# openclimatefix/predict_pv_yield

Measured on AMD Instinct MI355X. Metric: PV-site samples/sec (train step), conv3d 12->6 frames, higher is better.
Workload: dtype bf16; 1 GPU; conv3d train step (fwd + NMAE + bwd + Adam): sat [B,11,18,64,64] N(0,1), 4x Conv3d(3x3x3, 32ch) + fc 128/128/64, 128.6 M params; per_gpu_batch=32, global_batch=32, t_frames=18, parallelism=single

## Files before the change

include/pv_yield_hip.h:

```cpp
#ifndef PV_YIELD_HIP_H
#define PV_YIELD_HIP_H

#include <stddef.h>
#include <stdint.h>

#ifdef __cplusplus
extern "C" {
#endif

#define PV_ABI_VERSION 1

enum {
  PV_OK = 0,
  PV_EINVAL = -1,
  PV_ESIZE = -2,
  PV_ELAUNCH = -3
};

enum { PV_BORDER_CONSTANT = 0, PV_BORDER_REPLICATE = 1 };

enum {
  PV_U8_ROUND_DIV4 = 0,
  PV_U8_TRUNC_SCALE = 1
};
// ... 228 lines not shown

int pv_linear_f32_skinny_covers(int32_t m, int32_t n, int64_t k);
size_t pv_linear_fwd_f32_skinny_workspace_bytes(int32_t n);
int pv_linear_fwd_f32_skinny(const float* x, const float* w, const float* bias, float* y, int32_t m, int32_t n, int64_t k, int32_t relu,
                             void* workspace, size_t workspace_bytes, void* stream);
int pv_linear_dx_f32_skinny(const float* g, const float* w, float* dx, int32_t m, int32_t n, int64_t k, void* stream);

int pv_linear_workspace_bytes(int32_t m, int32_t n, int64_t k, size_t* bytes);
int pv_linear_fwd_f32(const float* x, const float* w, const float* bias, float* y,
                      int32_t m, int32_t n, int64_t k, int relu,
                      void* workspace, size_t workspace_bytes, void* stream);
int pv_linear_bwd_f32(const float* x, const float* w, const float* dy, const float* y_relu_mask,
                      float* dx, float* dw, float* db,
                      int32_t m, int32_t n, int64_t k, void* stream);

int pv_linear_bf16_workspace_bytes(int32_t m, int32_t n, int64_t k, size_t* bytes);
int pv_linear_fwd_bf16(const uint16_t* x, const uint16_t* w, const float* bias, float* y,
                       int32_t m, int32_t n, int64_t k, int relu,
                       void* workspace, size_t workspace_bytes, void* stream);
int pv_linear_bwd_bf16(const uint16_t* x, const uint16_t* w, const float* dy,
                       const float* y_relu_mask, uint16_t* dx, float* dw, float* db,
                       int32_t m, int32_t n, int64_t k, int32_t gate_dx_by_x, void* stream);

int pv_linear_wgrad_adam_bf16(const uint16_t* x, const float* dy, const float* y_relu_mask, float* param,
                              float* exp_avg, float* exp_avg_sq, uint16_t* bf16_shadow, int32_t m, int32_t n,
                              int64_t k, double lr, double beta1, double beta2, double eps, int32_t step,
                              void* stream);
int pv_linear_wgrad_adam_f32(const float* x, const float* dy, const float* y_relu_mask, float* param, float* exp_avg,
                             float* exp_avg_sq, int32_t m, int32_t n, int64_t k, double lr, double beta1, double beta2,
                             double eps, int32_t step, void* stream);
// ... 158 lines not shown
```

predict_pv_yield_amd/_lib.py:

```python
import ctypes
import os
import subprocess

_PKG = os.path.dirname(os.path.abspath(__file__))
LIB_PATH = os.environ.get("PV_YIELD_LIB") or os.path.join(_PKG, "lib", "libpvyield_hip.so")
CSRC_DIR = os.path.join(_PKG, "csrc")

PV_BORDER_CONSTANT = 0
PV_BORDER_REPLICATE = 1
PV_U8_ROUND_DIV4 = 0
PV_U8_TRUNC_SCALE = 1
PV_OPTFLOW_FARNEBACK_GAUSSIAN = 256

c_i32, c_i64, c_f32, c_f64 = ctypes.c_int32, ctypes.c_int64, ctypes.c_float, ctypes.c_double
c_vp, c_sz, c_int, c_u8 = ctypes.c_void_p, ctypes.c_size_t, ctypes.c_int, ctypes.c_uint8


class FarnebackParams(ctypes.Structure):
    _fields_ = [("pyr_scale", c_f64), ("levels", c_i32), ("winsize", c_i32), ("iterations", c_i32),
                ("poly_n", c_i32), ("poly_sigma", c_f64), ("flags", c_i32)]


class Conv3dDims(ctypes.Structure):
    _fields_ = [("batch", c_i32), ("c_in", c_i32), ("c_out", c_i32), ("t_in", c_i32), ("h_in", c_i32),
                ("w_in", c_i32), ("pad_t", c_i32), ("pad_h", c_i32), ("pad_w", c_i32)]

    def out_shape(self):
        return (self.t_in + 2 * self.pad_t - 2, self.h_in + 2 * self.pad_h - 2, self.w_in + 2 * self.pad_w - 2)


class AdamTensor(ctypes.Structure):
    _fields_ = [("param", c_vp), ("grad", c_vp), ("exp_avg", c_vp), ("exp_avg_sq", c_vp), ("bf16_shadow", c_vp),
                ("n", ctypes.c_uint64)]


class PackJob(ctypes.Structure):
    _fields_ = [("w", c_vp), ("wp", c_vp), ("c_out", c_i32), ("c_in", c_i32), ("transpose_flip", c_i32)]


class GemmDesc(ctypes.Structure):
    _fields_ = [("m", c_i32), ("n", c_i32), ("k", c_i32), ("a_rs", c_i64), ("a_cs", c_i64), ("b_rs", c_i64), ("b_cs", c_i64),
                ("ldc", c_i64), ("batch1", c_i32), ("batch2", c_i32), ("a_bs1", c_i64), ("a_bs2", c_i64), ("b_bs1", c_i64),
                ("b_bs2", c_i64), ("c_bs1", c_i64), ("c_bs2", c_i64), ("k_splits", c_i32), ("c_ss", c_i64)]


class AttentionDesc(ctypes.Structure):
    _fields_ = [("batch", c_i32), ("heads", c_i32), ("n_q", c_i32), ("n_k", c_i32), ("head_dim", c_i32),
                ("q_batch_stride", c_i64), ("q_row_stride", c_i64), ("k_batch_stride", c_i64), ("k_row_stride", c_i64),
                ("scale", c_f32)]


PV_ADAM_MAX_TENSORS = 32
PV_PACK_MAX_JOBS = 16


class Conv3dGeom(ctypes.Structure):
    _fields_ = [(n, c_i32) for n in ("batch", "c_in", "c_out", "t_in", "h_in", "w_in", "k_t", "k_h", "k_w",
                                     "stride_t", "stride_h", "stride_w", "pad_t", "pad_h", "pad_w")]

    def out_shape(self):
        return ((self.t_in + 2 * self.pad_t - self.k_t) // self.stride_t + 1,
                (self.h_in + 2 * self.pad_h - self.k_h) // self.stride_h + 1,
                (self.w_in + 2 * self.pad_w - self.k_w) // self.stride_w + 1)


_PFB = ctypes.POINTER(FarnebackParams)
_PCD = ctypes.POINTER(Conv3dDims)
_PCG = ctypes.POINTER(Conv3dGeom)
# ... 36 lines not shown
    "pv_conv3d_bwd_weight_bf16_workspace_bytes": [_PCD, ctypes.POINTER(c_sz)],
    "pv_conv3d_bwd_weight_bf16": [c_vp, c_vp, c_vp, c_vp, c_vp, _PCD, c_vp, c_sz, c_vp],
    "pv_conv3d_bwd_weight_f16": [c_vp, c_vp, c_vp, c_vp, _PCD, c_vp, c_sz, c_vp],
    "pv_conv3d_split2_weight_elems": [],
    "pv_conv3d_pack_weight_split2_f16": [c_vp, c_vp, c_vp, c_i32, c_i32, c_vp],
    "pv_conv3d_fwd_f16_f32out": [c_vp, c_vp, c_vp, c_i32, _PCD, c_vp],
    "pv_conv3d_fwd_f16_f32out_covers": [_PCD],
    "pv_sum3_ndhwc_to_ncdhw_f32": [c_vp, c_vp, c_vp, c_vp, c_i32, c_vp, c_vp, c_vp, c_vp, c_vp, c_vp, c_i32, c_i32, c_i64, c_vp],
    "pv_linear_f32_skinny_covers": [c_i32, c_i32, c_i64],
    "pv_linear_fwd_f32_skinny_workspace_bytes": [c_i32],
    "pv_linear_fwd_f32_skinny": [c_vp, c_vp, c_vp, c_vp, c_i32, c_i32, c_i64, c_i32, c_vp, c_sz, c_vp],
    "pv_linear_dx_f32_skinny": [c_vp, c_vp, c_vp, c_i32, c_i32, c_i64, c_vp],
    "pv_linear_workspace_bytes": [c_i32, c_i32, c_i64, ctypes.POINTER(c_sz)],
    "pv_linear_fwd_f32": [c_vp, c_vp, c_vp, c_vp, c_i32, c_i32, c_i64, c_int, c_vp, c_sz, c_vp],
    "pv_linear_bwd_f32": [c_vp, c_vp, c_vp, c_vp, c_vp, c_vp, c_vp, c_i32, c_i32, c_i64, c_vp],
    "pv_linear_bf16_workspace_bytes": [c_i32, c_i32, c_i64, ctypes.POINTER(c_sz)],
    "pv_linear_fwd_bf16": [c_vp, c_vp, c_vp, c_vp, c_i32, c_i32, c_i64, c_int, c_vp, c_sz, c_vp],
    "pv_linear_bwd_bf16": [c_vp, c_vp, c_vp, c_vp, c_vp, c_vp, c_vp, c_i32, c_i32, c_i64, c_i32, c_vp],
    "pv_linear_wgrad_adam_bf16": [c_vp, c_vp, c_vp, c_vp, c_vp, c_vp, c_vp, c_i32, c_i32, c_i64, c_f64, c_f64, c_f64, c_f64,
                                  c_i32, c_vp],
    "pv_linear_wgrad_adam_f32": [c_vp, c_vp, c_vp, c_vp, c_vp, c_vp, c_i32, c_i32, c_i64, c_f64, c_f64, c_f64, c_f64, c_i32, c_vp],
    "pv_linear_wgrad_dx_adam_bf16": [c_vp, c_vp, c_vp, c_vp, c_vp, c_vp, c_vp, c_vp, c_vp, c_i32, c_i32, c_i64, c_f64, c_f64,
                                     c_f64, c_f64, c_i32, c_i32, c_i32, c_vp],
    "pv_linear_wgrad_bf16out": [c_vp, c_vp, c_vp, c_vp, c_i32, c_i32, c_i64, c_vp],
    "pv_adam_step_bf16grad": [c_vp, c_vp, c_vp, c_vp, c_vp, c_sz, c_f64, c_f64, c_f64, c_f64, c_i32, c_f32, c_vp],
    "pv_conv3d_general_out_extent": [_PCG, _PI32, _PI32, _PI32],
    "pv_conv3d_general_fwd_f32": [c_vp, c_vp, c_vp, c_vp, _PCG, c_int, c_vp],
    "pv_conv3d_general_bwd_data_f32": [c_vp, c_vp, c_vp, c_vp, c_vp, _PCG, c_vp],
    "pv_conv3d_general_bwd_weight_workspace_bytes": [_PCG, ctypes.POINTER(c_sz)],
    "pv_conv3d_general_bwd_weight_f32": [c_vp, c_vp, c_vp, c_vp, c_vp, _PCG, c_vp, c_sz, c_vp],
# ... 161 lines not shown
```

predict_pv_yield_amd/csrc/dense_f32.hip:

```cpp
#include "pv_common.h"

namespace pv {

__global__ __launch_bounds__(256) void swap01_segments_kernel(const u32x4* __restrict__ src, u32x4* __restrict__ dst, long long n0,
                                                               long long n1, long long seg16) {
  const size_t total = (size_t)n0 * n1 * seg16, stride = (size_t)gridDim.x * blockDim.x;
  for (size_t i = (size_t)blockIdx.x * blockDim.x + threadIdx.x; i < total; i += stride) {
    const size_t seg = i / seg16, c = i - seg * seg16;
    const size_t i1 = seg / n0, i0 = seg - i1 * n0;
    dst[i] = src[(i0 * n1 + i1) * seg16 + c];
  }
}

constexpr int M_TILE = 8;
constexpr long long SMALL_K = 4096, SMALL_MN = 1 << 16;

__global__ __launch_bounds__(256) void linear_fwd_partial_f32(const float* __restrict__ x,
                                                               const float* __restrict__ w,
                                                               float* __restrict__ partial, int m, int n,
                                                               long long k, long long k_chunk) {
  const int col = blockIdx.x;
  const int ks = blockIdx.y;
  const int m0 = blockIdx.z * M_TILE;
  const long long k0 = (long long)ks * k_chunk;
  const long long k1 = k0 + k_chunk < k ? k0 + k_chunk : k;
  float acc[M_TILE];
#pragma unroll
  for (int i = 0; i < M_TILE; ++i) acc[i] = 0.f;
  const float* wr = w + (size_t)col * k;
// ... 105 lines not shown
  for (int ks = 0; ks < k_splits; ++ks) s += partial[(size_t)ks * m * n + i];
  if (bias) s += bias[col];
  if (relu) s = s > 0.f ? s : 0.f;
  y[i] = s;
}

__device__ __forceinline__ void linear_bwd_dx_body(float* g , const float* __restrict__ w,
                                                   const float* __restrict__ dy, const float* __restrict__ ymask,
                                                   float* __restrict__ dx, int m, int n, long long k, int bx, int by) {
  const int m0 = by * M_TILE;
  for (int i = threadIdx.x; i < n * M_TILE; i += blockDim.x) {
    int col = i / M_TILE, r = i % M_TILE;
    float v = 0.f;
    if (m0 + r < m) {
      size_t off = (size_t)(m0 + r) * n + col;
      v = dy[off];
      if (ymask && !(ymask[off] > 0.f)) v = 0.f;
    }
    g[i] = v;
  }
  __syncthreads();
  long long kk = (long long)bx * blockDim.x + threadIdx.x;
  if (kk >= k) return;
  float acc[M_TILE];
#pragma unroll
  for (int i = 0; i < M_TILE; ++i) acc[i] = 0.f;
  int col = 0;
  for (; col + 32 <= n; col += 32) {
    float wv[32];
#pragma unroll
    for (int j = 0; j < 32; ++j) wv[j] = w[(size_t)(col + j) * k + kk];
#pragma unroll
    for (int j = 0; j < 32; ++j)
#pragma unroll
      for (int i = 0; i < M_TILE; ++i) acc[i] = fmaf(g[(col + j) * M_TILE + i], wv[j], acc[i]);
  }
  for (; col + 8 <= n; col += 8) {
    float wv[8];
#pragma unroll
    for (int j = 0; j < 8; ++j) wv[j] = w[(size_t)(col + j) * k + kk];
#pragma unroll
    for (int j = 0; j < 8; ++j)
#pragma unroll
      for (int i = 0; i < M_TILE; ++i) acc[i] = fmaf(g[(col + j) * M_TILE + i], wv[j], acc[i]);
  }
  for (; col < n; ++col) {
    float wv = w[(size_t)col * k + kk];
#pragma unroll
    for (int i = 0; i < M_TILE; ++i) acc[i] = fmaf(g[col * M_TILE + i], wv, acc[i]);
  }
#pragma unroll
  for (int i = 0; i < M_TILE; ++i)
    if (m0 + i < m) dx[(size_t)(m0 + i) * k + kk] = acc[i];
}

__global__ __launch_bounds__(256) void linear_bwd_dx_f32(const float* __restrict__ w, const float* __restrict__ dy,
                                                          const float* __restrict__ ymask, float* __restrict__ dx,
                                                          int m, int n, long long k) {
  extern __shared__ float g[];
  linear_bwd_dx_body(g, w, dy, ymask, dx, m, n, k, blockIdx.x, blockIdx.y);
}

constexpr int N_TILE = 8;
__device__ __forceinline__ void linear_bwd_dw_body(float* g , const float* __restrict__ x,
                                                   const float* __restrict__ dy, const float* __restrict__ ymask,
                                                   float* __restrict__ dw, int m, int n, long long k, int bx, int by) {
  const int n0 = by * N_TILE;
  for (int i = threadIdx.x; i < m * N_TILE; i += blockDim.x) {
    int r = i / N_TILE, j = i % N_TILE;
    float v = 0.f;
    if (n0 + j < n) {
      size_t off = (size_t)r * n + n0 + j;
      v = dy[off];
      if (ymask && !(ymask[off] > 0.f)) v = 0.f;
    }
    g[i] = v;
  }
  __syncthreads();
  long long kk = (long long)bx * blockDim.x + threadIdx.x;
  if (kk >= k) return;
  float acc[N_TILE];
#pragma unroll
  for (int j = 0; j < N_TILE; ++j) acc[j] = 0.f;
  int r = 0;
  for (; r + 32 <= m; r += 32) {
    float xv[32];
#pragma unroll
    for (int q = 0; q < 32; ++q) xv[q] = x[(size_t)(r + q) * k + kk];
#pragma unroll
    for (int q = 0; q < 32; ++q)
#pragma unroll
      for (int j = 0; j < N_TILE; ++j) acc[j] = fmaf(g[(r + q) * N_TILE + j], xv[q], acc[j]);
  }
  for (; r + 8 <= m; r += 8) {
    float xv[8];
#pragma unroll
    for (int q = 0; q < 8; ++q) xv[q] = x[(size_t)(r + q) * k + kk];
#pragma unroll
    for (int q = 0; q < 8; ++q)
#pragma unroll
      for (int j = 0; j < N_TILE; ++j) acc[j] = fmaf(g[(r + q) * N_TILE + j], xv[q], acc[j]);
  }
  for (; r < m; ++r) {
    float xv = x[(size_t)r * k + kk];
#pragma unroll
    for (int j = 0; j < N_TILE; ++j) acc[j] = fmaf(g[r * N_TILE + j], xv, acc[j]);
  }
#pragma unroll
  for (int j = 0; j < N_TILE; ++j)
    if (n0 + j < n) dw[(size_t)(n0 + j) * k + kk] = acc[j];
}

__global__ __launch_bounds__(256) void linear_bwd_dw_f32(const float* __restrict__ x, const float* __restrict__ dy,
                                                          const float* __restrict__ ymask, float* __restrict__ dw,
                                                          int m, int n, long long k) {
  extern __shared__ float g[];
  linear_bwd_dw_body(g, x, dy, ymask, dw, m, n, k, blockIdx.x, blockIdx.y);
}

__device__ __forceinline__ void linear_bwd_db_body(const float* __restrict__ dy, const float* __restrict__ ymask,
                                                   float* __restrict__ db, int m, int n, int bx);

__global__ __launch_bounds__(256) void linear_bwd_db_f32(const float* __restrict__ dy, const float* __restrict__ ymask,
                                                          float* __restrict__ db, int m, int n) {
  linear_bwd_db_body(dy, ymask, db, m, n, blockIdx.x);
}

__device__ __forceinline__ void linear_bwd_db_body(const float* __restrict__ dy, const float* __restrict__ ymask,
                                                   float* __restrict__ db, int m, int n, int bx) {
  int col = bx * blockDim.x + threadIdx.x;
  if (col >= n) return;
  float s = 0.f;
  for (int r = 0; r < m; ++r) {
    size_t off = (size_t)r * n + col;
    float v = dy[off];
    if (ymask && !(ymask[off] > 0.f)) v = 0.f;
    s += v;
  }
  db[col] = s;
}

__global__ __launch_bounds__(256) void linear_bwd_small_f32(const float* __restrict__ x, const float* __restrict__ w,
                                                             const float* __restrict__ dy, const float* __restrict__ ymask,
                                                             float* __restrict__ dx, float* __restrict__ dw,
                                                             float* __restrict__ db, int m, int n, long long k, int kb,
                                                             int n_dx, int n_dw) {
  extern __shared__ float g[];
  int blk = blockIdx.x;
  if (blk < n_dx) {
    linear_bwd_dx_body(g, w, dy, ymask, dx, m, n, k, blk % kb, blk / kb);
  } else if (blk < n_dx + n_dw) {
    blk -= n_dx;
    linear_bwd_dw_body(g, x, dy, ymask, dw, m, n, k, blk % kb, blk / kb);
  } else {
    linear_bwd_db_body(dy, ymask, db, m, n, blk - n_dx - n_dw);
  }
}

__global__ __launch_bounds__(256) void linear_fwd_small_f32(const float* __restrict__ x, const float* __restrict__ w,
                                                             const float* __restrict__ bias, float* __restrict__ y, int m,
                                                             int n, int k, int relu) {
  const int i = blockIdx.x * blockDim.x + threadIdx.x;
  if (i >= m * n) return;
  const int r = i / n, col = i - r * n;
  const float* xr = x + (size_t)r * k;
  const float* wr = w + (size_t)col * k;
  float s0 = 0.f, s1 = 0.f, s2 = 0.f, s3 = 0.f;
  int kk = 0;
  if ((((uintptr_t)xr | (uintptr_t)wr) & 15) == 0) {
    for (; kk + 64 <= k; kk += 64) {
      f32x4 xv[16], wv[16];
#pragma unroll
      for (int j = 0; j < 16; ++j) xv[j] = *reinterpret_cast<const f32x4*>(xr + kk + 4 * j), wv[j] = *reinterpret_cast<const f32x4*>(wr + kk + 4 * j);
#pragma unroll
      for (int j = 0; j < 16; ++j) {
        s0 = fmaf(xv[j][0], wv[j][0], s0);
        s1 = fmaf(xv[j][1], wv[j][1], s1);
        s2 = fmaf(xv[j][2], wv[j][2], s2);
        s3 = fmaf(xv[j][3], wv[j][3], s3);
      }
    }
    for (; kk + 32 <= k; kk += 32) {
      f32x4 xv[8], wv[8];
#pragma unroll
      for (int j = 0; j < 8; ++j) xv[j] = *reinterpret_cast<const f32x4*>(xr + kk + 4 * j), wv[j] = *reinterpret_cast<const f32x4*>(wr + kk + 4 * j);
#pragma unroll
      for (int j = 0; j < 8; ++j) {
        s0 = fmaf(xv[j][0], wv[j][0], s0);
        s1 = fmaf(xv[j][1], wv[j][1], s1);
        s2 = fmaf(xv[j][2], wv[j][2], s2);
        s3 = fmaf(xv[j][3], wv[j][3], s3);
      }
    }
  }
  for (; kk + 4 <= k; kk += 4) {
    s0 = fmaf(xr[kk], wr[kk], s0);
    s1 = fmaf(xr[kk + 1], wr[kk + 1], s1);
    s2 = fmaf(xr[kk + 2], wr[kk + 2], s2);
    s3 = fmaf(xr[kk + 3], wr[kk + 3], s3);
  }
  for (; kk < k; ++kk) s0 = fmaf(xr[kk], wr[kk], s0);
  float s = (s0 + s1) + (s2 + s3);
  if (bias) s += bias[col];
  if (relu) s = s > 0.f ? s : 0.f;
  y[i] = s;
}

struct LossWeights { float w[64]; };

__global__ __launch_bounds__(256) void forecast_losses_f32(const float* __restrict__ y_hat, const float* __restrict__ y,
                                                            long long y_row_stride, long long y_col_stride, int m,
                                                            int n, float grad_scale, LossWeights lw,
                                                            float* __restrict__ out4, float* __restrict__ grad,
                                                            float* __restrict__ per_horizon) {
  float s_se = 0.f, s_ae = 0.f, s_wse = 0.f, s_wae = 0.f;
  const int total = m * n;
  const float inv = 1.0f / (float)total;
  for (int i = threadIdx.x; i < total; i += blockDim.x) {
    int r = i / n, c = i - r * n;
    float d = y_hat[i] - y[(long long)r * y_row_stride + (long long)c * y_col_stride];
// ... 480 lines not shown
```

predict_pv_yield_amd/functional.py:

```python
import ctypes

import torch

from . import hip_ops as K
from ._lib import check, current_stream_ptr, get_lib, ptr


LINEAR_F32_GEMM_K = 1 << 16
F32_PENDING_MAX_ROWS = 1024


def exact_f32() -> bool:
    import os
    return bool(os.environ.get("PV_EXACT_F32"))


class LinearF32(torch.autograd.Function):
    @staticmethod
    def forward(ctx, x, weight, bias, relu):
        x = x.contiguous()
        if (not exact_f32() and x.dtype == torch.float32 and weight.is_contiguous()
                and K.linear_f32_skinny_covers(x.shape[0], weight.shape[0], x.shape[1])):
            y = K.linear_fwd_f32_skinny(x, weight, bias.contiguous() if bias is not None else None, relu)
        else:
# ... 24 lines not shown
                dw = None
            else:
                if earlier is not None:
                    x0, g0 = earlier
                    owner._pv_pending_f32 = None
                    dw0 = K.gemm(g0.t(), x0)
                    owner.grad = dw0 if owner.grad is None else owner.grad + dw0
                dw = K.gemm(g.t(), x)
            return dx, dw, (K.colsum(g) if ctx.has_bias else None), None
        dx, dw, db = K.linear_bwd_f32(x, weight.contiguous(), dy.contiguous(), y, need_dx=ctx.needs_input_grad[0])
        return dx, dw, (db if ctx.has_bias else None), None


def linear_f32(x, weight, bias, relu=False):
    return LinearF32.apply(x, weight, bias, relu)


USE_RELU_MASKS = True


class PackInputBF16(torch.autograd.Function):

    @staticmethod
    def forward(ctx, x):
        out = K.pack_ncdhw_f32_to_ndhwc_bf16(x.contiguous())
        ctx.mark_non_differentiable(out)
        return out

    @staticmethod
    def backward(ctx, g):
# ... 566 lines not shown
```

predict_pv_yield_amd/hip_ops.py:

```python
import ctypes
from typing import Optional, Sequence

import numpy as np
import torch

from . import _lib
from ._lib import (Conv3dDims, Conv3dGeom, FarnebackParams, PV_BORDER_CONSTANT, PV_BORDER_REPLICATE,
                   PV_OPTFLOW_FARNEBACK_GAUSSIAN, check, current_stream_ptr, get_lib, ptr, require_cuda)

c_i32, c_i64, c_f32, c_f64, c_sz = ctypes.c_int32, ctypes.c_int64, ctypes.c_float, ctypes.c_double, ctypes.c_size_t


def u8_from_10bit(x: torch.Tensor, mode: int = 0, return_flag: bool = False):
    require_cuda(x)
    out = torch.empty(x.shape, dtype=torch.uint8, device=x.device)
    flag = torch.zeros(1, dtype=torch.int32, device=x.device)
    lib = get_lib()
    if x.dtype == torch.int16:
        fn = lib.pv_u8_from_10bit_i16
    elif x.dtype == torch.float32:
        fn = lib.pv_u8_from_10bit_f32
    else:
        raise TypeError(f"u8_from_10bit: int16 or float32 expected, got {x.dtype}")
    check(fn(ptr(x), ptr(out), x.numel(), mode, ptr(flag), current_stream_ptr()), "pv_u8_from_10bit")
# ... 557 lines not shown
    dx = torch.empty((m, k), dtype=torch.float32, device=g.device)
    check(get_lib().pv_linear_dx_f32_skinny(ptr(g), ptr(weight), ptr(dx), m, n, k, current_stream_ptr()), "pv_linear_dx_f32_skinny")
    return dx


def linear_bwd_f32(x, weight, dy, y_mask, need_dx=True):
    require_cuda(x, weight, dy, y_mask)
    m, k = x.shape
    n = weight.shape[0]
    dx = torch.empty((m, k), dtype=torch.float32, device=x.device) if need_dx else None
    dw = torch.empty((n, k), dtype=torch.float32, device=x.device)
    db = torch.empty(n, dtype=torch.float32, device=x.device)
    check(get_lib().pv_linear_bwd_f32(ptr(x), ptr(weight), ptr(dy), ptr(y_mask), ptr(dx), ptr(dw), ptr(db), m, n, k,
                                      current_stream_ptr()), "pv_linear_bwd_f32")
    return dx, dw, db


LINEAR_FWD_MAX_ROWS = 1024


def linear_fwd_bf16(x_bf16, w_bf16, bias, relu=False):
    require_cuda(x_bf16, w_bf16, bias)
    m, k = x_bf16.shape
    n = w_bf16.shape[0]
    need = c_sz(0)
    lib = get_lib()
    cap = LINEAR_FWD_MAX_ROWS if (32 <= n <= 128 and n % 16 == 0) else 128
    check(lib.pv_linear_bf16_workspace_bytes(min(m, cap), n, k, ctypes.byref(need)), "pv_linear_bf16_workspace_bytes")
    ws = _workspace("linear_bf16", need.value, x_bf16.device)
    y = torch.empty((m, n), dtype=torch.float32, device=x_bf16.device)
# ... 1214 lines not shown
```

predict_pv_yield_amd/models/conv3d/model.py:

```python
import logging

import torch
from torch import nn

from ...data.batch import BatchML
from ..base_model import BaseModel

logging.basicConfig()
_LOG = logging.getLogger("predict_pv_yield_amd")


FC1_CHANNELS_LAST = True


class Model(BaseModel):

    name = "conv3d"

    def __init__(
        self,
        include_pv_yield: bool = True,
        include_nwp: bool = True,
        forecast_minutes: int = 30,
        history_minutes: int = 60,
# ... 102 lines not shown
            return replace_future_frames_with_flow(sat.float(), n_future=self.forecast_len_5)
        return sat.float()

    def forward(self, x):
        if type(x) == dict:
            x = BatchML(**x)
        sat_data = self._satellite_input(x)
        from ... import functional as Fn
        from ._tower import conv_tower_fc1
        self._mark_fc1_layout()

        batch_size = sat_data.shape[0]
        out = conv_tower_fc1(sat_data, self._conv_layers(), self.fc1, self.number_sat_channels, self.conv3d_channels,
                             (0, 0, 0), self.cnn_output_size, self.precision == "bf16" and self._bf16_supported(),
                             fc1_channels_last=bool(self._fc1_k_channels))
        out = Fn.linear_f32(out, self.fc2.weight, self.fc2.bias, relu=True)

        if self.include_pv_yield:
            pv_yield_history = x[self.output_variable][:, : self.history_len_30 + 1].nan_to_num(nan=0.0).float()
            pv_yield_history = pv_yield_history.reshape(pv_yield_history.shape[0],
                                                        pv_yield_history.shape[1] * pv_yield_history.shape[2])
            out = torch.cat((out, pv_yield_history), dim=1)
        if self.include_nwp:
            nwp_data = x["nwp"].float().flatten(start_dim=1)
            out_nwp = Fn.linear_f32(nwp_data, self.fc_nwp.weight, self.fc_nwp.bias, relu=True)
            out = torch.cat((out, out_nwp), dim=1)

        out = Fn.linear_f32(out, self.fc3.weight, self.fc3.bias, relu=True)
        out = Fn.linear_f32(out, self.fc4.weight, self.fc4.bias, relu=False)
        return out.reshape(batch_size, self.forecast_len)
# ... 1 lines not shown
```

Measured before the change: 20330 samples/s.

## Fuse fc2/fc3/fc4 MLP head into single forward and backward kernels

Adds fused HIP kernels that run the three small fp32 linear layers after fc1 in one launch for the forward pass and one for the backward pass. Activations stay in LDS between layers, and the backward kernel computes the dx chain, dw and db tiles together. The goal is to cut per-layer kernel-launch and autograd overhead for the tiny batch-32 head. The model uses this path only when neither PV-yield history nor NWP inputs are included, and it falls back to per-layer linears when the shapes do not fit in LDS. The existing dense kernels are refactored into shared device bodies.

New measurement: 20620 samples/s (median of 6 runs). 1.01x the previous value.

```diff
diff --git a/include/pv_yield_hip.h b/include/pv_yield_hip.h
--- a/include/pv_yield_hip.h
+++ b/include/pv_yield_hip.h
@@ -266,6 +266,21 @@
                       float* dx, float* dw, float* db,
                       int32_t m, int32_t n, int64_t k, void* stream);
 
+#define PV_MLP_HEAD_MAX_LAYERS 3
+typedef struct pv_mlp_layer {
+  const float* w;
+  const float* bias;
+  float* y;
+  float* dw;
+  float* db;
+  int32_t n;
+  int32_t relu;
+} pv_mlp_layer;
+int pv_mlp_head_max_rows(int32_t k1, const int32_t* n, int32_t n_layers);
+int pv_mlp_head_fwd_f32(const float* x, int32_t m, int32_t k1, const pv_mlp_layer* layers, int32_t n_layers, void* stream);
+int pv_mlp_head_bwd_f32(const float* x, const float* dy, float* dx, int32_t m, int32_t k1, const pv_mlp_layer* layers,
+                        int32_t n_layers, void* stream);
+
 int pv_linear_bf16_workspace_bytes(int32_t m, int32_t n, int64_t k, size_t* bytes);
 int pv_linear_fwd_bf16(const uint16_t* x, const uint16_t* w, const float* bias, float* y,
                        int32_t m, int32_t n, int64_t k, int relu,
diff --git a/predict_pv_yield_amd/_lib.py b/predict_pv_yield_amd/_lib.py
--- a/predict_pv_yield_amd/_lib.py
+++ b/predict_pv_yield_amd/_lib.py
@@ -38,6 +38,10 @@
     _fields_ = [("w", c_vp), ("wp", c_vp), ("c_out", c_i32), ("c_in", c_i32), ("transpose_flip", c_i32)]
 
 
+class MlpLayer(ctypes.Structure):
+    _fields_ = [("w", c_vp), ("bias", c_vp), ("y", c_vp), ("dw", c_vp), ("db", c_vp), ("n", c_i32), ("relu", c_i32)]
+
+
 class GemmDesc(ctypes.Structure):
     _fields_ = [("m", c_i32), ("n", c_i32), ("k", c_i32), ("a_rs", c_i64), ("a_cs", c_i64), ("b_rs", c_i64), ("b_cs", c_i64),
                 ("ldc", c_i64), ("batch1", c_i32), ("batch2", c_i32), ("a_bs1", c_i64), ("a_bs2", c_i64), ("b_bs1", c_i64),
@@ -52,6 +56,7 @@
 
 PV_ADAM_MAX_TENSORS = 32
 PV_PACK_MAX_JOBS = 16
+PV_MLP_HEAD_MAX_LAYERS = 3
 
 
 class Conv3dGeom(ctypes.Structure):
@@ -118,6 +123,9 @@
     "pv_linear_workspace_bytes": [c_i32, c_i32, c_i64, ctypes.POINTER(c_sz)],
     "pv_linear_fwd_f32": [c_vp, c_vp, c_vp, c_vp, c_i32, c_i32, c_i64, c_int, c_vp, c_sz, c_vp],
     "pv_linear_bwd_f32": [c_vp, c_vp, c_vp, c_vp, c_vp, c_vp, c_vp, c_i32, c_i32, c_i64, c_vp],
+    "pv_mlp_head_max_rows": [c_i32, _PI32, c_i32],
+    "pv_mlp_head_fwd_f32": [c_vp, c_i32, c_i32, ctypes.POINTER(MlpLayer), c_i32, c_vp],
+    "pv_mlp_head_bwd_f32": [c_vp, c_vp, c_vp, c_i32, c_i32, ctypes.POINTER(MlpLayer), c_i32, c_vp],
     "pv_linear_bf16_workspace_bytes": [c_i32, c_i32, c_i64, ctypes.POINTER(c_sz)],
     "pv_linear_fwd_bf16": [c_vp, c_vp, c_vp, c_vp, c_i32, c_i32, c_i64, c_int, c_vp, c_sz, c_vp],
     "pv_linear_bwd_bf16": [c_vp, c_vp, c_vp, c_vp, c_vp, c_vp, c_vp, c_i32, c_i32, c_i64, c_i32, c_vp],
diff --git a/predict_pv_yield_amd/csrc/dense_f32.hip b/predict_pv_yield_amd/csrc/dense_f32.hip
--- a/predict_pv_yield_amd/csrc/dense_f32.hip
+++ b/predict_pv_yield_amd/csrc/dense_f32.hip
@@ -1,4 +1,5 @@
 #include "pv_common.h"
+#include "dense_f32_bodies.h"
 
 namespace pv {
 
@@ -12,7 +13,6 @@
   }
 }
 
-constexpr int M_TILE = 8;
 constexpr long long SMALL_K = 4096, SMALL_MN = 1 << 16;
 
 __global__ __launch_bounds__(256) void linear_fwd_partial_f32(const float* __restrict__ x,
@@ -148,8 +148,7 @@
     float v = 0.f;
     if (m0 + r < m) {
       size_t off = (size_t)(m0 + r) * n + col;
-      v = dy[off];
-      if (ymask && !(ymask[off] > 0.f)) v = 0.f;
+      v = linear_bwd_gate(dy[off], ymask, off);
     }
     g[i] = v;
   }
@@ -157,32 +156,7 @@
   long long kk = (long long)bx * blockDim.x + threadIdx.x;
   if (kk >= k) return;
   float acc[M_TILE];
-#pragma unroll
-  for (int i = 0; i < M_TILE; ++i) acc[i] = 0.f;
-  int col = 0;
-  for (; col + 32 <= n; col += 32) {
-    float wv[32];
-#pragma unroll
-    for (int j = 0; j < 32; ++j) wv[j] = w[(size_t)(col + j) * k + kk];
-#pragma unroll
-    for (int j = 0; j < 32; ++j)
-#pragma unroll
-      for (int i = 0; i < M_TILE; ++i) acc[i] = fmaf(g[(col + j) * M_TILE + i], wv[j], acc[i]);
-  }
-  for (; col + 8 <= n; col += 8) {
-    float wv[8];
-#pragma unroll
-    for (int j = 0; j < 8; ++j) wv[j] = w[(size_t)(col + j) * k + kk];
-#pragma unroll
-    for (int j = 0; j < 8; ++j)
-#pragma unroll
-      for (int i = 0; i < M_TILE; ++i) acc[i] = fmaf(g[(col + j) * M_TILE + i], wv[j], acc[i]);
-  }
-  for (; col < n; ++col) {
-    float wv = w[(size_t)col * k + kk];
-#pragma unroll
-    for (int i = 0; i < M_TILE; ++i) acc[i] = fmaf(g[col * M_TILE + i], wv, acc[i]);
-  }
+  linear_bwd_dx_acc<M_TILE>(g, M_TILE, w, n, k, kk, acc);
 #pragma unroll
   for (int i = 0; i < M_TILE; ++i)
     if (m0 + i < m) dx[(size_t)(m0 + i) * k + kk] = acc[i];
@@ -195,7 +169,6 @@
   linear_bwd_dx_body(g, w, dy, ymask, dx, m, n, k, blockIdx.x, blockIdx.y);
 }
 
-constexpr int N_TILE = 8;
 __device__ __forceinline__ void linear_bwd_dw_body(float* g , const float* __restrict__ x,
                                                    const float* __restrict__ dy, const float* __restrict__ ymask,
                                                    float* __restrict__ dw, int m, int n, long long k, int bx, int by) {
@@ -205,8 +178,7 @@
     float v = 0.f;
     if (n0 + j < n) {
       size_t off = (size_t)r * n + n0 + j;
-      v = dy[off];
-      if (ymask && !(ymask[off] > 0.f)) v = 0.f;
+      v = linear_bwd_gate(dy[off], ymask, off);
     }
     g[i] = v;
   }
@@ -214,32 +186,7 @@
   long long kk = (long long)bx * blockDim.x + threadIdx.x;
   if (kk >= k) return;
   float acc[N_TILE];
-#pragma unroll
-  for (int j = 0; j < N_TILE; ++j) acc[j] = 0.f;
-  int r = 0;
-  for (; r + 32 <= m; r += 32) {
-    float xv[32];
-#pragma unroll
-    for (int q = 0; q < 32; ++q) xv[q] = x[(size_t)(r + q) * k + kk];
-#pragma unroll
-    for (int q = 0; q < 32; ++q)
-#pragma unroll
-      for (int j = 0; j < N_TILE; ++j) acc[j] = fmaf(g[(r + q) * N_TILE + j], xv[q], acc[j]);
-  }
-  for (; r + 8 <= m; r += 8) {
-    float xv[8];
-#pragma unroll
-    for (int q = 0; q < 8; ++q) xv[q] = x[(size_t)(r + q) * k + kk];
-#pragma unroll
-    for (int q = 0; q < 8; ++q)
-#pragma unroll
-      for (int j = 0; j < N_TILE; ++j) acc[j] = fmaf(g[(r + q) * N_TILE + j], xv[q], acc[j]);
-  }
-  for (; r < m; ++r) {
-    float xv = x[(size_t)r * k + kk];
-#pragma unroll
-    for (int j = 0; j < N_TILE; ++j) acc[j] = fmaf(g[r * N_TILE + j], xv, acc[j]);
-  }
+  linear_bwd_dw_acc(g, x, m, k, kk, acc);
 #pragma unroll
   for (int j = 0; j < N_TILE; ++j)
     if (n0 + j < n) dw[(size_t)(n0 + j) * k + kk] = acc[j];
@@ -264,14 +211,10 @@
                                                    float* __restrict__ db, int m, int n, int bx) {
   int col = bx * blockDim.x + threadIdx.x;
   if (col >= n) return;
-  float s = 0.f;
-  for (int r = 0; r < m; ++r) {
-    size_t off = (size_t)r * n + col;
-    float v = dy[off];
-    if (ymask && !(ymask[off] > 0.f)) v = 0.f;
-    s += v;
-  }
-  db[col] = s;
+  db[col] = linear_bwd_db_sum(m, [&](int r) {
+    const size_t off = (size_t)r * n + col;
+    return linear_bwd_gate(dy[off], ymask, off);
+  });
 }
 
 __global__ __launch_bounds__(256) void linear_bwd_small_f32(const float* __restrict__ x, const float* __restrict__ w,
@@ -299,45 +242,7 @@
   const int r = i / n, col = i - r * n;
   const float* xr = x + (size_t)r * k;
   const float* wr = w + (size_t)col * k;
-  float s0 = 0.f, s1 = 0.f, s2 = 0.f, s3 = 0.f;
-  int kk = 0;
-  if ((((uintptr_t)xr | (uintptr_t)wr) & 15) == 0) {
-    for (; kk + 64 <= k; kk += 64) {
-      f32x4 xv[16], wv[16];
-#pragma unroll
-      for (int j = 0; j < 16; ++j) xv[j] = *reinterpret_cast<const f32x4*>(xr + kk + 4 * j), wv[j] = *reinterpret_cast<const f32x4*>(wr + kk + 4 * j);
-#pragma unroll
-      for (int j = 0; j < 16; ++j) {
-        s0 = fmaf(xv[j][0], wv[j][0], s0);
-        s1 = fmaf(xv[j][1], wv[j][1], s1);
-        s2 = fmaf(xv[j][2], wv[j][2], s2);
-        s3 = fmaf(xv[j][3], wv[j][3], s3);
-      }
-    }
-    for (; kk + 32 <= k; kk += 32) {
-      f32x4 xv[8], wv[8];
-#pragma unroll
-      for (int j = 0; j < 8; ++j) xv[j] = *reinterpret_cast<const f32x4*>(xr + kk + 4 * j), wv[j] = *reinterpret_cast<const f32x4*>(wr + kk + 4 * j);
-#pragma unroll
-      for (int j = 0; j < 8; ++j) {
-        s0 = fmaf(xv[j][0], wv[j][0], s0);
-        s1 = fmaf(xv[j][1], wv[j][1], s1);
-        s2 = fmaf(xv[j][2], wv[j][2], s2);
-        s3 = fmaf(xv[j][3], wv[j][3], s3);
-      }
-    }
-  }
-  for (; kk + 4 <= k; kk += 4) {
-    s0 = fmaf(xr[kk], wr[kk], s0);
-    s1 = fmaf(xr[kk + 1], wr[kk + 1], s1);
-    s2 = fmaf(xr[kk + 2], wr[kk + 2], s2);
-    s3 = fmaf(xr[kk + 3], wr[kk + 3], s3);
-  }
-  for (; kk < k; ++kk) s0 = fmaf(xr[kk], wr[kk], s0);
-  float s = (s0 + s1) + (s2 + s3);
-  if (bias) s += bias[col];
-  if (relu) s = s > 0.f ? s : 0.f;
-  y[i] = s;
+  y[i] = linear_fwd_epilogue_f32(linear_fwd_dot_f32(xr, wr, k), bias, col, relu);
 }
 
 struct LossWeights { float w[64]; };
diff --git a/predict_pv_yield_amd/csrc/dense_f32_bodies.h b/predict_pv_yield_amd/csrc/dense_f32_bodies.h
--- /dev/null
+++ b/predict_pv_yield_amd/csrc/dense_f32_bodies.h
@@ -0,0 +1,126 @@
+#pragma once
+#include "pv_common.h"
+
+namespace pv {
+
+constexpr int M_TILE = 8;
+constexpr int N_TILE = 8;
+
+__device__ __forceinline__ float linear_fwd_dot_f32(const float* __restrict__ xr, const float* __restrict__ wr, int k) {
+  float s0 = 0.f, s1 = 0.f, s2 = 0.f, s3 = 0.f;
+  int kk = 0;
+  if ((((uintptr_t)xr | (uintptr_t)wr) & 15) == 0) {
+    for (; kk + 64 <= k; kk += 64) {
+      f32x4 xv[16], wv[16];
+#pragma unroll
+      for (int j = 0; j < 16; ++j) xv[j] = *reinterpret_cast<const f32x4*>(xr + kk + 4 * j), wv[j] = *reinterpret_cast<const f32x4*>(wr + kk + 4 * j);
+#pragma unroll
+      for (int j = 0; j < 16; ++j) {
+        s0 = fmaf(xv[j][0], wv[j][0], s0);
+        s1 = fmaf(xv[j][1], wv[j][1], s1);
+        s2 = fmaf(xv[j][2], wv[j][2], s2);
+        s3 = fmaf(xv[j][3], wv[j][3], s3);
+      }
+    }
+    for (; kk + 32 <= k; kk += 32) {
+      f32x4 xv[8], wv[8];
+#pragma unroll
+      for (int j = 0; j < 8; ++j) xv[j] = *reinterpret_cast<const f32x4*>(xr + kk + 4 * j), wv[j] = *reinterpret_cast<const f32x4*>(wr + kk + 4 * j);
+#pragma unroll
+      for (int j = 0; j < 8; ++j) {
+        s0 = fmaf(xv[j][0], wv[j][0], s0);
+        s1 = fmaf(xv[j][1], wv[j][1], s1);
+        s2 = fmaf(xv[j][2], wv[j][2], s2);
+        s3 = fmaf(xv[j][3], wv[j][3], s3);
+      }
+    }
+  }
+  for (; kk + 4 <= k; kk += 4) {
+    s0 = fmaf(xr[kk], wr[kk], s0);
+    s1 = fmaf(xr[kk + 1], wr[kk + 1], s1);
+    s2 = fmaf(xr[kk + 2], wr[kk + 2], s2);
+    s3 = fmaf(xr[kk + 3], wr[kk + 3], s3);
+  }
+  for (; kk < k; ++kk) s0 = fmaf(xr[kk], wr[kk], s0);
+  return (s0 + s1) + (s2 + s3);
+}
+
+__device__ __forceinline__ float linear_fwd_epilogue_f32(float s, const float* __restrict__ bias, int col, int relu) {
+  if (bias) s += bias[col];
+  if (relu) s = s > 0.f ? s : 0.f;
+  return s;
+}
+
+__device__ __forceinline__ float linear_bwd_gate(float dy, const float* __restrict__ ymask, size_t off) {
+  return (ymask && !(ymask[off] > 0.f)) ? 0.f : dy;
+}
+
+template <int R>
+__device__ __forceinline__ void linear_bwd_dx_acc(const float* g, int g_stride, const float* __restrict__ w, int n, long long k,
+                                                  long long kk, float (&acc)[R]) {
+#pragma unroll
+  for (int i = 0; i < R; ++i) acc[i] = 0.f;
+  int col = 0;
+  for (; col + 32 <= n; col += 32) {
+    float wv[32];
+#pragma unroll
+    for (int j = 0; j < 32; ++j) wv[j] = w[(size_t)(col + j) * k + kk];
+#pragma unroll
+    for (int j = 0; j < 32; ++j)
+#pragma unroll
+      for (int i = 0; i < R; ++i) acc[i] = fmaf(g[(col + j) * g_stride + i], wv[j], acc[i]);
+  }
+  for (; col + 8 <= n; col += 8) {
+    float wv[8];
+#pragma unroll
+    for (int j = 0; j < 8; ++j) wv[j] = w[(size_t)(col + j) * k + kk];
+#pragma unroll
+    for (int j = 0; j < 8; ++j)
+#pragma unroll
+      for (int i = 0; i < R; ++i) acc[i] = fmaf(g[(col + j) * g_stride + i], wv[j], acc[i]);
+  }
+  for (; col < n; ++col) {
+    float wv = w[(size_t)col * k + kk];
+#pragma unroll
+    for (int i = 0; i < R; ++i) acc[i] = fmaf(g[col * g_stride + i], wv, acc[i]);
+  }
+}
+
+__device__ __forceinline__ void linear_bwd_dw_acc(const float* g, const float* __restrict__ x, int m, long long k, long long kk,
+                                                  float (&acc)[N_TILE]) {
+#pragma unroll
+  for (int j = 0; j < N_TILE; ++j) acc[j] = 0.f;
+  int r = 0;
+  for (; r + 32 <= m; r += 32) {
+    float xv[32];
+#pragma unroll
+    for (int q = 0; q < 32; ++q) xv[q] = x[(size_t)(r + q) * k + kk];
+#pragma unroll
+    for (int q = 0; q < 32; ++q)
+#pragma unroll
+      for (int j = 0; j < N_TILE; ++j) acc[j] = fmaf(g[(r + q) * N_TILE + j], xv[q], acc[j]);
+  }
+  for (; r + 8 <= m; r += 8) {
+    float xv[8];
+#pragma unroll
+    for (int q = 0; q < 8; ++q) xv[q] = x[(size_t)(r + q) * k + kk];
+#pragma unroll
+    for (int q = 0; q < 8; ++q)
+#pragma unroll
+      for (int j = 0; j < N_TILE; ++j) acc[j] = fmaf(g[(r + q) * N_TILE + j], xv[q], acc[j]);
+  }
+  for (; r < m; ++r) {
+    float xv = x[(size_t)r * k + kk];
+#pragma unroll
+    for (int j = 0; j < N_TILE; ++j) acc[j] = fmaf(g[r * N_TILE + j], xv, acc[j]);
+  }
+}
+
+template <class G>
+__device__ __forceinline__ float linear_bwd_db_sum(int m, G g_at) {
+  float s = 0.f;
+  for (int r = 0; r < m; ++r) s += g_at(r);
+  return s;
+}
+
+}
diff --git a/predict_pv_yield_amd/csrc/mlp_head_f32.hip b/predict_pv_yield_amd/csrc/mlp_head_f32.hip
--- /dev/null
+++ b/predict_pv_yield_amd/csrc/mlp_head_f32.hip
@@ -0,0 +1,239 @@
+#include "pv_common.h"
+#include "dense_f32_bodies.h"
+
+namespace pv {
+
+constexpr int HEAD_MAX_LAYERS = PV_MLP_HEAD_MAX_LAYERS;
+constexpr int HEAD_MAX_WIDTH = 4096;
+constexpr int HEAD_DX_ROWS = 2;
+constexpr long long HEAD_MAX_MN = 1 << 16;
+constexpr size_t HEAD_MAX_LDS = 64 * 1024;
+
+struct HeadArgs {
+  pv_mlp_layer layer[HEAD_MAX_LAYERS];
+  int n_layers;
+};
+
+__global__ __launch_bounds__(256) void mlp_head_fwd_f32_kernel(const float* __restrict__ x, HeadArgs a, int m, int k1,
+                                                               int rows_per_wg, int ws) {
+  extern __shared__ __attribute__((aligned(16))) float head_lds[];
+  const int r0 = blockIdx.x * rows_per_wg;
+  const int rows = m - r0 < rows_per_wg ? m - r0 : rows_per_wg;
+  float* cur = head_lds;
+  float* nxt = head_lds + (size_t)rows_per_wg * ws;
+  for (int i = threadIdx.x; i < rows * k1; i += blockDim.x) {
+    const int r = i / k1, c = i - r * k1;
+    cur[r * ws + c] = x[(size_t)(r0 + r) * k1 + c];
+  }
+  __syncthreads();
+  int k = k1;
+  for (int l = 0; l < a.n_layers; ++l) {
+    const pv_mlp_layer L = a.layer[l];
+    for (int i = threadIdx.x; i < rows * L.n; i += blockDim.x) {
+      const int r = i / L.n, col = i - r * L.n;
+      const float s = linear_fwd_epilogue_f32(linear_fwd_dot_f32(cur + r * ws, L.w + (size_t)col * k, k), L.bias, col, L.relu);
+      L.y[(size_t)(r0 + r) * L.n + col] = s;
+      nxt[r * ws + col] = s;
+    }
+    __syncthreads();
+    float* t = cur; cur = nxt; nxt = t;
+    k = L.n;
+  }
+}
+
+template <class Out>
+__device__ __forceinline__ void head_dx_stage(const float* G, int n, const float* __restrict__ w, int k, int rows, int c0, int cn,
+                                              Out out) {
+  for (int it = threadIdx.x; it < rows * cn; it += blockDim.x) {
+    const int r = it / cn, kk = c0 + (it - r * cn);
+    float acc[1];
+    linear_bwd_dx_acc<1>(G + (size_t)r * n, 1, w, n, (long long)k, (long long)kk, acc);
+    out(r, kk, acc[0]);
+  }
+}
+
+__device__ __forceinline__ const float* head_mask(const pv_mlp_layer& L) { return L.relu ? L.y : nullptr; }
+
+__device__ __forceinline__ const float* head_g_chain(const HeadArgs& a, const float* __restrict__ dy, int ra, int rows, int stop,
+                                                     float* Ga, float* Gb) {
+  const int last = a.n_layers - 1;
+  {
+    const pv_mlp_layer L = a.layer[last];
+    const float* mask = head_mask(L);
+    for (int i = threadIdx.x; i < rows * L.n; i += blockDim.x) {
+      const size_t off = (size_t)ra * L.n + i;
+      Ga[i] = linear_bwd_gate(dy[off], mask, off);
+    }
+  }
+  __syncthreads();
+  for (int j = last; j > stop; --j) {
+    const pv_mlp_layer L = a.layer[j], P = a.layer[j - 1];
+    const float* mask = head_mask(P);
+    float* Gout = Gb;
+    head_dx_stage(Ga, L.n, L.w, P.n, rows, 0, P.n, [&](int r, int kk, float v) {
+      Gout[r * P.n + kk] = linear_bwd_gate(v, mask, (size_t)(ra + r) * P.n + kk);
+    });
+    __syncthreads();
+    float* t = Ga; Ga = Gb; Gb = t;
+  }
+  return Ga;
+}
+
+struct HeadBwdPlan {
+  int n_dx;
+  int tile0[HEAD_MAX_LAYERS + 1];
+  int kb[HEAD_MAX_LAYERS];
+  int g_floats;
+};
+
+__global__ __launch_bounds__(256) void mlp_head_bwd_f32_kernel(const float* __restrict__ x, const float* __restrict__ dy,
+                                                               float* __restrict__ dx, HeadArgs a, HeadBwdPlan p, int m, int k1) {
+  extern __shared__ __attribute__((aligned(16))) float head_lds[];
+  float* Ga = head_lds;
+  float* Gb = head_lds + p.g_floats;
+  float* gt = head_lds + 2 * (size_t)p.g_floats;
+  const int blk = blockIdx.x;
+  if (blk < p.n_dx) {
+    const int ra = blk * HEAD_DX_ROWS;
+    const int rows = m - ra < HEAD_DX_ROWS ? m - ra : HEAD_DX_ROWS;
+    const float* G = head_g_chain(a, dy, ra, rows, 0, Ga, Gb);
+    const pv_mlp_layer L = a.layer[0];
+    head_dx_stage(G, L.n, L.w, k1, rows, 0, k1, [&](int r, int kk, float v) { dx[(size_t)(ra + r) * k1 + kk] = v; });
+    return;
+  }
+  int t = 0;
+  while (t + 1 < a.n_layers && blk - p.n_dx >= p.tile0[t + 1]) ++t;
+  const pv_mlp_layer L = a.layer[t];
+  const int tile = blk - p.n_dx - p.tile0[t];
+  const int bx = tile % p.kb[t], n0 = (tile / p.kb[t]) * N_TILE;
+  const int k = t == 0 ? k1 : a.layer[t - 1].n;
+  const float* xin = t == 0 ? x : a.layer[t - 1].y;
+  const float* mask = head_mask(L);
+  if (t == a.n_layers - 1) {
+    for (int i = threadIdx.x; i < m * N_TILE; i += blockDim.x) {
+      const int r = i / N_TILE, j = i % N_TILE;
+      float v = 0.f;
+      if (n0 + j < L.n) {
+        const size_t off = (size_t)r * L.n + n0 + j;
+        v = linear_bwd_gate(dy[off], mask, off);
+      }
+      gt[i] = v;
+    }
+  } else {
+    const float* G = head_g_chain(a, dy, 0, m, t + 1, Ga, Gb);
+    const pv_mlp_layer U = a.layer[t + 1];
+    const int cn = L.n - n0 < N_TILE ? L.n - n0 : N_TILE;
+    if (cn < N_TILE)
+      for (int i = threadIdx.x; i < m * N_TILE; i += blockDim.x)
+        if (i % N_TILE >= cn) gt[i] = 0.f;
+    head_dx_stage(G, U.n, U.w, L.n, m, n0, cn, [&](int r, int kk, float v) {
+      gt[r * N_TILE + (kk - n0)] = linear_bwd_gate(v, mask, (size_t)r * L.n + kk);
+    });
+  }
+  __syncthreads();
+  if (bx == 0 && threadIdx.x < N_TILE && n0 + (int)threadIdx.x < L.n) {
+    const int j = threadIdx.x;
+    L.db[n0 + j] = linear_bwd_db_sum(m, [&](int r) { return gt[r * N_TILE + j]; });
+  }
+  const long long kk = (long long)bx * blockDim.x + threadIdx.x;
+  if (kk >= k) return;
+  float acc[N_TILE];
+  linear_bwd_dw_acc(gt, xin, m, (long long)k, kk, acc);
+#pragma unroll
+  for (int j = 0; j < N_TILE; ++j)
+    if (n0 + j < L.n) L.dw[(size_t)(n0 + j) * k + kk] = acc[j];
+}
+
+static int head_args(const pv_mlp_layer* layers, int32_t n_layers, int32_t m, int32_t k1, HeadArgs* a, const char* who) {
+  PV_REQUIRE(layers && n_layers >= 1 && n_layers <= HEAD_MAX_LAYERS, PV_EINVAL, "%s: 1..%d layers", who, HEAD_MAX_LAYERS);
+  PV_REQUIRE(m > 0 && k1 > 0 && k1 <= HEAD_MAX_WIDTH, PV_ESIZE, "%s: m > 0 and k1 in 1..%d, got %d x %d", who, HEAD_MAX_WIDTH, m, k1);
+  a->n_layers = n_layers;
+  for (int l = 0; l < n_layers; ++l) {
+    PV_REQUIRE(layers[l].w && layers[l].y, PV_EINVAL, "%s: null weight / output of layer %d", who, l);
+    PV_REQUIRE(layers[l].n > 0 && layers[l].n <= HEAD_MAX_WIDTH, PV_ESIZE, "%s: layer %d has %d outputs (1..%d)", who, l,
+               layers[l].n, HEAD_MAX_WIDTH);
+    PV_REQUIRE((long long)m * layers[l].n <= HEAD_MAX_MN, PV_ESIZE, "%s: %d rows x %d outputs of layer %d is no small layer", who, m,
+               layers[l].n, l);
+    a->layer[l] = layers[l];
+  }
+  return PV_OK;
+}
+
+static size_t head_bwd_g_floats(const HeadArgs& a, int m) {
+  int wide_all = 0, wide_upper = 0;
+  for (int l = 0; l < a.n_layers; ++l) {
+    wide_all = std::max(wide_all, a.layer[l].n);
+    if (l > 0) wide_upper = std::max(wide_upper, a.layer[l].n);
+  }
+  return (std::max((size_t)m * wide_upper, (size_t)HEAD_DX_ROWS * wide_all) + 3) & ~(size_t)3;
+}
+
+}
+
+using namespace pv;
+
+extern "C" {
+
+int pv_mlp_head_max_rows(int32_t k1, const int32_t* n, int32_t n_layers) {
+  if (!n || n_layers < 1 || n_layers > HEAD_MAX_LAYERS || k1 < 1 || k1 > HEAD_MAX_WIDTH) return 0;
+  HeadArgs a;
+  a.n_layers = n_layers;
+  for (int l = 0; l < n_layers; ++l) {
+    if (n[l] < 1 || n[l] > HEAD_MAX_WIDTH) return 0;
+    a.layer[l].n = n[l];
+  }
+  int wide = 1;
+  for (int l = 0; l < n_layers; ++l) wide = std::max(wide, n[l]);
+  int lo = 0, hi = (int)(HEAD_MAX_MN / wide);
+  while (lo < hi) {
+    const int mid = (lo + hi + 1) / 2;
+    if ((2 * head_bwd_g_floats(a, mid) + (size_t)mid * N_TILE) * sizeof(float) <= HEAD_MAX_LDS) lo = mid; else hi = mid - 1;
+  }
+  return lo;
+}
+
+int pv_mlp_head_fwd_f32(const float* x, int32_t m, int32_t k1, const pv_mlp_layer* layers, int32_t n_layers, void* stream) {
+  HeadArgs a;
+  const int rc = head_args(layers, n_layers, m, k1, &a, "pv_mlp_head_fwd_f32");
+  if (rc) return rc;
+  PV_REQUIRE(x, PV_EINVAL, "pv_mlp_head_fwd_f32: null x");
+  int wide = k1;
+  for (int l = 0; l < n_layers; ++l) wide = std::max(wide, a.layer[l].n);
+  const int ws = (wide + 3) & ~3;
+  const int rows_per_wg = (m + kNumCU - 1) / kNumCU;
+  const size_t lds = 2 * (size_t)rows_per_wg * ws * sizeof(float);
+  PV_REQUIRE(lds <= HEAD_MAX_LDS, PV_ESIZE, "pv_mlp_head_fwd_f32: %d rows of %d features do not fit the LDS image", m, wide);
+  const unsigned threads = (unsigned)std::min(256, ((rows_per_wg * std::max(wide, 64)) + 63) & ~63);
+  hipLaunchKernelGGL(mlp_head_fwd_f32_kernel, dim3((unsigned)((m + rows_per_wg - 1) / rows_per_wg)), dim3(threads), lds,
+                     as_stream(stream), x, a, m, k1, rows_per_wg, ws);
+  return check_launch("pv_mlp_head_fwd_f32");
+}
+
+int pv_mlp_head_bwd_f32(const float* x, const float* dy, float* dx, int32_t m, int32_t k1, const pv_mlp_layer* layers,
+                        int32_t n_layers, void* stream) {
+  HeadArgs a;
+  const int rc = head_args(layers, n_layers, m, k1, &a, "pv_mlp_head_bwd_f32");
+  if (rc) return rc;
+  PV_REQUIRE(x && dy, PV_EINVAL, "pv_mlp_head_bwd_f32: null x / dy");
+  HeadBwdPlan p;
+  p.n_dx = dx ? (m + HEAD_DX_ROWS - 1) / HEAD_DX_ROWS : 0;
+  int tiles = 0;
+  for (int l = 0; l < n_layers; ++l) {
+    PV_REQUIRE(a.layer[l].dw && a.layer[l].db, PV_EINVAL, "pv_mlp_head_bwd_f32: null dw / db of layer %d", l);
+    const int k = l == 0 ? k1 : a.layer[l - 1].n;
+    p.kb[l] = (k + 255) / 256;
+    p.tile0[l] = tiles;
+    tiles += p.kb[l] * ((a.layer[l].n + N_TILE - 1) / N_TILE);
+  }
+  for (int l = n_layers; l <= HEAD_MAX_LAYERS; ++l) p.tile0[l] = tiles;
+  for (int l = n_layers; l < HEAD_MAX_LAYERS; ++l) p.kb[l] = 1;
+  const size_t g_floats = head_bwd_g_floats(a, m);
+  const size_t lds = (2 * g_floats + (size_t)m * N_TILE) * sizeof(float);
+  PV_REQUIRE(lds <= HEAD_MAX_LDS, PV_ESIZE, "pv_mlp_head_bwd_f32: %d rows do not fit the LDS images (pv_mlp_head_max_rows)", m);
+  p.g_floats = (int)g_floats;
+  hipLaunchKernelGGL(mlp_head_bwd_f32_kernel, dim3((unsigned)(p.n_dx + tiles)), dim3(256), lds, as_stream(stream), x, dy, dx, a, p,
+                     m, k1);
+  return check_launch("pv_mlp_head_bwd_f32");
+}
+
+}
diff --git a/predict_pv_yield_amd/functional.py b/predict_pv_yield_amd/functional.py
--- a/predict_pv_yield_amd/functional.py
+++ b/predict_pv_yield_amd/functional.py
@@ -62,6 +62,56 @@
 
 def linear_f32(x, weight, bias, relu=False):
     return LinearF32.apply(x, weight, bias, relu)
+
+
+MLP_HEAD_MAX_ROWS = 64
+SMALL_LINEAR_K = 4096
+
+
+class MlpHeadF32(torch.autograd.Function):
+
+    @staticmethod
+    def forward(ctx, x, relus, *params):
+        x = x.contiguous()
+        layers = [(params[2 * i].contiguous(), None if params[2 * i + 1] is None else params[2 * i + 1].contiguous(), bool(r))
+                  for i, r in enumerate(relus)]
+        ys = K.mlp_head_fwd(x, layers)
+        ctx.relus = tuple(relus)
+        ctx.has_bias = [b is not None for _, b, _ in layers]
+        ctx.save_for_backward(x, *[w for w, _, _ in layers], *ys)
+        return ys[-1]
+
+    @staticmethod
+    def backward(ctx, dy):
+        n = len(ctx.relus)
+        x, ws, ys = ctx.saved_tensors[0], ctx.saved_tensors[1:1 + n], ctx.saved_tensors[1 + n:]
+        layers = [(w, None, r) for w, r in zip(ws, ctx.relus)]
+        dx, grads = K.mlp_head_bwd(x, dy.contiguous(), layers, list(ys), need_dx=ctx.needs_input_grad[0])
+        out = [dx, None]
+        for (dw, db), has_bias in zip(grads, ctx.has_bias):
+            out += [dw, db if has_bias else None]
+        return tuple(out)
+
+
+def mlp_head_covers(x, layers) -> bool:
+    if x.dtype != torch.float32 or x.dim() != 2 or not x.is_cuda or exact_f32():
+        return False
+    m, k = x.shape
+    if m < 1 or m > MLP_HEAD_MAX_ROWS or any(w.dtype != torch.float32 or w.dim() != 2 for w, _, _ in layers):
+        return False
+    ks = [k] + [w.shape[0] for w, _, _ in layers]
+    if any(w.shape[1] != kin for (w, _, _), kin in zip(layers, ks)) or max(ks) > SMALL_LINEAR_K:
+        return False
+    return m <= K.mlp_head_max_rows(k, ks[1:])
+
+
+def mlp_head_f32(x, layers):
+    if mlp_head_covers(x, layers):
+        flat = [t for w, b, _ in layers for t in (w, b)]
+        return MlpHeadF32.apply(x, tuple(bool(r) for _, _, r in layers), *flat)
+    for w, b, relu in layers:
+        x = linear_f32(x, w, b, relu=relu)
+    return x
 
 
 USE_RELU_MASKS = True
diff --git a/predict_pv_yield_amd/hip_ops.py b/predict_pv_yield_amd/hip_ops.py
--- a/predict_pv_yield_amd/hip_ops.py
+++ b/predict_pv_yield_amd/hip_ops.py
@@ -595,6 +595,53 @@
     check(get_lib().pv_linear_bwd_f32(ptr(x), ptr(weight), ptr(dy), ptr(y_mask), ptr(dx), ptr(dw), ptr(db), m, n, k,
                                       current_stream_ptr()), "pv_linear_bwd_f32")
     return dx, dw, db
+
+
+def _mlp_head_shapes(x, layers, who):
+    if x.dim() != 2 or x.dtype != torch.float32 or not 1 <= len(layers) <= _lib.PV_MLP_HEAD_MAX_LAYERS:
+        raise TypeError(f"{who}: float32 x [M, K] and 1..{_lib.PV_MLP_HEAD_MAX_LAYERS} layers expected")
+    m, k = x.shape
+    ns = []
+    for i, (w, b, _) in enumerate(layers):
+        require_cuda(w, b)
+        if w.dtype != torch.float32 or w.dim() != 2 or w.shape[1] != k or (b is not None and (b.dtype != torch.float32 or tuple(b.shape) != (w.shape[0],))):
+            raise TypeError(f"{who}: layer {i} needs a float32 weight [n, {k}] and bias [n], got {tuple(w.shape)} / "
+                            f"{None if b is None else tuple(b.shape)}")
+        k = w.shape[0]
+        ns.append(k)
+    return m, x.shape[1], ns
+
+
+def mlp_head_max_rows(k1: int, ns: Sequence[int]) -> int:
+    if not 1 <= len(ns) <= _lib.PV_MLP_HEAD_MAX_LAYERS:
+        return 0
+    return int(get_lib().pv_mlp_head_max_rows(int(k1), (c_i32 * len(ns))(*[int(n) for n in ns]), len(ns)))
+
+
+def mlp_head_fwd(x, layers):
+    require_cuda(x)
+    m, k1, ns = _mlp_head_shapes(x, layers, "mlp_head_fwd")
+    ys = [torch.empty((m, n), dtype=torch.float32, device=x.device) for n in ns]
+    arr = (_lib.MlpLayer * len(layers))()
+    for i, ((w, b, relu), y) in enumerate(zip(layers, ys)):
+        arr[i] = _lib.MlpLayer(ptr(w), ptr(b), ptr(y), None, None, ns[i], int(bool(relu)))
+    check(get_lib().pv_mlp_head_fwd_f32(ptr(x), m, k1, arr, len(layers), current_stream_ptr()), "pv_mlp_head_fwd_f32")
+    return ys
+
+
+def mlp_head_bwd(x, dy, layers, ys, need_dx=True):
+    require_cuda(x, dy, *ys)
+    m, k1, ns = _mlp_head_shapes(x, layers, "mlp_head_bwd")
+    if dy.dtype != torch.float32 or tuple(dy.shape) != (m, ns[-1]) or [tuple(y.shape) for y in ys] != [(m, n) for n in ns]:
+        raise TypeError(f"mlp_head_bwd: dy [{m}, {ns[-1]}] and one stored output per layer expected")
+    dx = torch.empty((m, k1), dtype=torch.float32, device=x.device) if need_dx else None
+    grads = [(torch.empty_like(w), torch.empty(w.shape[0], dtype=torch.float32, device=x.device)) for w, _, _ in layers]
+    arr = (_lib.MlpLayer * len(layers))()
+    for i, ((w, b, relu), y, (dw, db)) in enumerate(zip(layers, ys, grads)):
+        arr[i] = _lib.MlpLayer(ptr(w), ptr(b), ptr(y), ptr(dw), ptr(db), ns[i], int(bool(relu)))
+    check(get_lib().pv_mlp_head_bwd_f32(ptr(x), ptr(dy), ptr(dx), m, k1, arr, len(layers), current_stream_ptr()),
+          "pv_mlp_head_bwd_f32")
+    return dx, grads
 
 
 LINEAR_FWD_MAX_ROWS = 1024
diff --git a/predict_pv_yield_amd/models/conv3d/model.py b/predict_pv_yield_amd/models/conv3d/model.py
--- a/predict_pv_yield_amd/models/conv3d/model.py
+++ b/predict_pv_yield_amd/models/conv3d/model.py
@@ -140,6 +140,10 @@
         out = conv_tower_fc1(sat_data, self._conv_layers(), self.fc1, self.number_sat_channels, self.conv3d_channels,
                              (0, 0, 0), self.cnn_output_size, self.precision == "bf16" and self._bf16_supported(),
                              fc1_channels_last=bool(self._fc1_k_channels))
+        if not (self.include_pv_yield or self.include_nwp):
+            out = Fn.mlp_head_f32(out, [(self.fc2.weight, self.fc2.bias, True), (self.fc3.weight, self.fc3.bias, True),
+                                        (self.fc4.weight, self.fc4.bias, False)])
+            return out.reshape(batch_size, self.forecast_len)
         out = Fn.linear_f32(out, self.fc2.weight, self.fc2.bias, relu=True)
 
         if self.include_pv_yield:
```
